# theteamatx/x-edr-trajectory-planning

Hardware: AMD Instinct MI355X
Metric: time-optimal path timings/s (7-DOF, 2000 s-samples), 1/2/4/8 MI355X + %HBM roofline (higher is better)
Workload: dtype f64

## Files before the change

### x-edr-trajectory-planning_amd/csrc/tpamd_sweep_joint.h

```cpp
#pragma once

#include <type_traits>

#include "tpamd_kernels.h"

namespace tpamd {

__device__ __forceinline__ double uniform_f64(double v) {
  const int lo = __builtin_amdgcn_readfirstlane(__double2loint(v));
  const int hi = __builtin_amdgcn_readfirstlane(__double2hiint(v));
  return __hiloint2double(hi, lo);
}
__device__ __forceinline__ double readlane_f64(double v, int lane) {
  const int lo = __builtin_amdgcn_readlane(__double2loint(v), lane);
  const int hi = __builtin_amdgcn_readlane(__double2hiint(v), lane);
  return __hiloint2double(hi, lo);
}
__device__ __forceinline__ int uniform_i32(int v) { return __builtin_amdgcn_readfirstlane(v); }
__device__ __forceinline__ int lds_word(const int *p) {
  return *(const volatile __attribute__((address_space(3))) int *)p;
}

template <int CTRL>
__device__ __forceinline__ double dpp_f64(double v) {
// ... 88 lines not shown
__device__ __forceinline__ double ordered_sum64_finite(double t, double d, const OrderedSumMasks &k) {
  double acc = t;
  const double one = 1.0;
  asm volatile("s_nop 1" ::: "memory");
  TPAMD_OSM_ROW("0x1");
  ordered_sum_carry<1>(acc);
  TPAMD_OSM_ROW("0x2");
  ordered_sum_carry<2>(acc);
  TPAMD_OSM_ROW("0x4");
  ordered_sum_carry<3>(acc);
  TPAMD_OSM_ROW("0x8");
  return acc;
}

#ifdef TPAMD_DIAG
__device__ __forceinline__ long long tpamd_stamp() {
  unsigned long long t;
  __builtin_amdgcn_sched_barrier(0);
  asm volatile("s_memtime %0\n\ts_waitcnt lgkmcnt(0)" : "=s"(t)::"memory");
  __builtin_amdgcn_sched_barrier(0);
  return (long long)t;
}
#define TPAMD_T0(var) const long long var = tpamd_stamp()
#ifdef TPAMD_DIAG_REASONS
#define TPAMD_ACC(slot, var) do { if (!((slot) == 12 || (slot) == 13 || (slot) == 17 || ((slot) >= 19 && (slot) <= 23) || (slot) == 31)) diag[slot] += tpamd_stamp() - (var); } while (0)
#else
#define TPAMD_ACC(slot, var) diag[slot] += tpamd_stamp() - (var)
#endif
#define TPAMD_CNT(slot) diag[slot] += 1
#define TPAMD_ADD(slot, v) diag[slot] += (v)
#define TPAMD_CNTX(slot) diagx[slot] += 1
#define TPAMD_T0C(var) const long long var = tpamd_stamp()
#define TPAMD_ACCC(slot, var) diag[slot] += tpamd_stamp() - (var)
#ifdef TPAMD_DIAG_LIGHT
#undef TPAMD_T0
#undef TPAMD_ACC
#define TPAMD_T0(var)
#define TPAMD_ACC(slot, var)
#endif
#else
#define TPAMD_T0(var)
#define TPAMD_ACC(slot, var)
#define TPAMD_T0C(var)
#define TPAMD_ACCC(slot, var)
#define TPAMD_CNT(slot)
#define TPAMD_ADD(slot, v)
#define TPAMD_CNTX(slot)
#endif

#ifndef TPAMD_TILE_SAMPLES
#define TPAMD_TILE_SAMPLES 32
#endif
#ifndef TPAMD_CHAIN_GUESS
#define TPAMD_CHAIN_GUESS 0
#endif
#ifndef TPAMD_CURVE_EXIT
#define TPAMD_CURVE_EXIT 1
#endif
constexpr int kTileSamples = TPAMD_TILE_SAMPLES;
template <int D>
struct TileCfg {
  static constexpr int kSamples = (D > 8 && TPAMD_TILE_SAMPLES > 16) ? 16 : TPAMD_TILE_SAMPLES;
};

typedef double f64x2 __attribute__((ext_vector_type(2)));

template <int K>
struct RegPack {
  f64x2 v;
  RegPack<K - 1> rest;
  template <int LIMIT>
  __device__ __forceinline__ void load(const f64x2 *src, int c) {
    if (c < LIMIT) v = src[c];
    rest.template load<LIMIT>(src, c + 64);
  }
  template <int LIMIT>
  __device__ __forceinline__ void store(f64x2 *dst, int c) const {
// ... 13 lines not shown
  static constexpr int RPL = (D + PARTS - 1) / PARTS;
  static constexpr int kCandLanes = 2 * D * PARTS;
  static constexpr int kRows16 = (kCandLanes + 15) / 16;
  static_assert(kCandLanes <= 64, "candidate lanes must fit one wave");
#ifndef TPAMD_CHAIN_STEPS
#define TPAMD_CHAIN_STEPS 16
#endif
  static constexpr int kChain = TPAMD_CHAIN_STEPS;
  static constexpr int GRP = 64 / kChain;
  static constexpr int CPL = (2 * D + GRP - 1) / GRP;
  static constexpr int VPL = (D + GRP - 1) / GRP;
  static constexpr unsigned long long kPart0 =
      (GRP == 4) ? 0x1111111111111111ull : ((GRP == 2) ? 0x5555555555555555ull : ~0ull);
  static_assert(GRP == 1 || GRP == 2 || GRP == 4, "chain steps must be 16, 32 or 64");
};

template <bool MAX>
__device__ __forceinline__ double ext2(double a, double b) {
  return ext2_raw<MAX>(a, b);
}

template <int D, int E = 0>
struct JointSweep {
  typedef JointLayout<D> L;
  static_assert(E == 0 || E == 2, "extra rows come as one pair");
  static constexpr int R = 2 * D + E + 2;
  static constexpr int kMt = D + E / 2;
  static constexpr int kTile = TileCfg<D>::kSamples;
  static constexpr int kChunks = kTile * R / 2;
  static constexpr int kChunksPerLane = (kChunks + 63) / 64;
#ifdef TPAMD_DIAG
  long long diag[32];
  mutable long long diagx[kDiagExt];
#endif
  int N, lane;
  double ds, two_ds;
  double *sd2;
  double *tiles;
  const uint8_t *typel;
  double *sdd_g;
  const double *m_g;
  const double *rec;
  int tag0, tag1;
  double *qd_g, *qdd_g;
  const double *aml;
  uint32_t *dirty;
  int end_idx;
  double lim;
  double chk_hi[L::RPL];
  double vel_hi;
  double vel_lo;
  int vel_mode;
  double ex_hi[E ? E : 1];
  int own_off;
  int chk_off[L::RPL];
  int vel_off;
  double row_lo, row_hi;
  double v_lim[L::CPL];
  int v_off[L::CPL];
  double vv_hi[L::VPL];
  double va_hi[L::VPL];
  int vv_off[L::VPL];

  struct Rows {
    f64x2 own;
    f64x2 chk[L::RPL];
// ... 604 lines not shown
    load_rows(idx, rows);
    if (load_cur) c.cur = uniform_f64(sd2[idx]);
    double m0, m1;
    int t0, t1;
    load_mt(idx, m0, t0);
    load_mt(idx + dir, m1, t1);
    c.m_i = uniform_f64(m0); c.m_n = uniform_f64(m1);
    c.t_i = uniform_i32(t0); c.t_n = uniform_i32(t1);
    c.nxt = uniform_f64(sd2[idx + dir]);
    c.win = -1;
    TPAMD_ACC(26, ti_);
  }

  template <bool FWD>
  __device__ __forceinline__ int add_extremal(int idx_start, Prefetch &pf, bool pair_signal = false,
                                              bool wait_pair = false) {
#define TPAMD_PAIR_SIGNAL()                                   \
  do {                                                        \
    if (pair_signal) {                                        \
      __threadfence_block();                                  \
      __syncthreads();                                        \
      pair_signal = false;                                    \
    }                                                         \
  } while (0)
    if (FWD ? !(idx_start < N - 2) : !(idx_start > 1)) {
      end_idx = idx_start;
      TPAMD_PAIR_SIGNAL();
      if (wait_pair) __syncthreads();
      return FWD ? N - 1 : 0;
    }
    Rows rows_a, rows_b;
    Carry c;
    init_carry<FWD>(idx_start, c, rows_a, pf, true);
    if (wait_pair && is_tiny(c.cur - c.m_i) && (c.t_i & kBndTrajectory) && (c.t_n & kBndTrajectory)) {
      __syncthreads();
      wait_pair = false;
    }
    bool trust = true;
    int last_win = -1;
    for (;;) {
#define TPAMD_TRY_FOLLOW()                                                                   \
  if (is_tiny(c.cur - c.m_i) && (c.t_i & kBndTrajectory) && (c.t_n & kBndTrajectory)) {      \
    TPAMD_T0(tfb_);                                                                          \
    const int run = uniform_i32(follow_boundary<FWD>(c));                                    \
    TPAMD_ACC(25, tfb_);                                                                     \
    if (run > 0) {                                                                           \
      TPAMD_CNT(8);                                                                          \
      TPAMD_PAIR_SIGNAL();                                                                   \
      if (FWD ? !(c.idx < N - 2) : !(c.idx > 1)) {                                           \
        end_idx = c.idx;                                                                     \
        return FWD ? N - 1 : 0;                                                              \
      }                                                                                      \
      init_carry<FWD>(c.idx, c, rows_a, pf, false);                                          \
      continue;                                                                              \
    }                                                                                        \
  }
#define TPAMD_TRY_CHAIN()                                                                    \
  if (c.win >= 0 && (trust || c.win == last_win)) {                                          \
    int total = 0, run, next_win;                                                            \
    bool again, curve;                                                                       \
    do {                                                                                     \
      { TPAMD_T0(tc_); run = uniform_i32(follow_chain<FWD>(c, pf, next_win, curve)); TPAMD_ACC(4, tc_); } \
      TPAMD_CNT(6);                                                                          \
      total += run;                                                                          \
      again = run == L::kChain;                                                              \
       \
// ... 66 lines not shown
    for (int top = idx_hi; top >= 1; top -= 256) {
      uint8_t ty[4];
#pragma unroll
      for (int u = 0; u < 4; u++) ty[u] = typel[max(top - 64 * u - lane, 0)];
#pragma unroll
      for (int u = 0; u < 4; u++) {
        const int idx = top - 64 * u - lane;
        const unsigned long long m = __ballot((idx >= 1) & ((ty[u] & kBndEqualsZ00) != 0));
        if (m) return top - 64 * u - (__ffsll((long long)m) - 1);
      }
    }
    return -1;
  }

#ifdef TPAMD_DIAG
  __device__ __forceinline__ int next_critical_point_literal(int idx_lo, int idx_hi) const {
    int crit = -1;
    for (int idx = idx_lo + 1; idx <= idx_hi; idx++) {
      if (crit < 0) {
        if (typel[idx] & (kBndSource | kBndTrajectory)) crit = idx;
      } else if (typel[idx] & kBndEqualsZ00) {
        crit = idx;
      }
      if (crit > 0 && !isnan(sd2[idx])) return crit;
    }
    return -1;
  }
#endif
};

constexpr int kRefitCap = 128;
constexpr int kRefitLdsBytes = kRefitCap * (4 + 8 + 8);

template <int D, int E>
struct PathBoundary {
  const JointSource &src;
  const Workspace &ws;
  int b, N, stride, lane;
  size_t pb;
  double ds, z00;
  const uint8_t *at_l;
  uint8_t *ff_l, *typel;
  bool keep;
  int *l_idx;
  double *l_val, *l_nxt;
  int count;

  __device__ __forceinline__ void append(bool need, int j, double val, double nxt) {
    const unsigned long long mask = __ballot(need);
    if (!mask) return;
    if (need) {
      const int pos = count + __popcll(mask & ((1ull << lane) - 1ull));
      l_idx[pos] = j;
      l_val[pos] = val;
      l_nxt[pos] = nxt;
    }
    count += __popcll(mask);
  }

  __device__ __forceinline__ void refit_one(int j, double sd2v, double *x, double *y) const {
    constexpr int R = 2 * D + E + 2;
    const f64x2 *rec2 = reinterpret_cast<const f64x2 *>(src.q12 + ((size_t)b * stride + j) * R);
    const double *lim_lo = src.lim + (size_t)b * 2 * (2 * D + E), *lim_hi = lim_lo + 2 * D + E;
    double a[D], bq[D];
#pragma unroll
    for (int d = 0; d < D; d++) {
      const f64x2 p = rec2[d];
      a[d] = p.x;
      bq[d] = p.y;
    }
    bool ok = true;
    if (E > 0) {
      const f64x2 ex = rec2[D];
      const double vt = ex.x * sd2v, vr = ex.y * sd2v;
      ok = !(vt + kTiny < lim_lo[2 * D] || vt - kTiny > lim_hi[2 * D]) &&
           !(vr + kTiny < lim_lo[2 * D + 1] || vr - kTiny > lim_hi[2 * D + 1]);
    }
    if (ok) find_sdd_both_joint_fixed<D>(a, bq, lim_hi, sd2v, x, y);
  }

  __device__ __forceinline__ void finalize(int j, double m, double X, double Y, double m_next) const {
    uint8_t type = kBndNone;
    if (j >= 1 && j <= N - 2) {
      const double sd2p = (m_next - m) / ds;
      const double sd2p_min = 2 * Y;
      const double sd2p_max = 2 * X;
      if (sd2p < sd2p_min) type = kBndSink;
      else if (sd2p > sd2p_max) type = kBndSource;
      if ((sd2p <= sd2p_max) && (sd2p >= sd2p_min)) type = kBndTrajectory;
    }
    if (m == z00) type |= kBndEqualsZ00;
    ws.m[pb + j] = m;
    typel[j] = type;
    if (keep) {
      ws.X[pb + j] = X;
      ws.Y[pb + j] = Y;
      ws.type[pb + j] = type;
    }
  }

  template <bool FINAL>
  __device__ __forceinline__ void flush(long long *diag) {
    TPAMD_T0(tf);
    __builtin_amdgcn_fence(__ATOMIC_ACQ_REL, "wavefront");
    __builtin_amdgcn_wave_barrier();
    const int n = count;
    for (int e = lane; e < n; e += 64) {
      const int j = l_idx[e];
      const double val = l_val[e];
      double x = 0.0, y = 0.0;
      refit_one(j, val, &x, &y);
      if (FINAL) finalize(j, val, x, y, l_nxt[e]);
      else { ws.Xz[pb + j] = x; ws.Yz[pb + j] = y; }
    }
    count = 0;
    __builtin_amdgcn_fence(__ATOMIC_ACQ_REL, "wavefront");
    __builtin_amdgcn_wave_barrier();
    if (FINAL) TPAMD_ACC(23, tf);
  }
};

template <int D, int E>
__device__ __forceinline__ void boundary_passes_for_path(const JointSource &src, const Workspace &ws, int b,
                                                         int N, int stride, int tid, uint8_t *at_l,
                                                         uint8_t *ff_l, char *scratch, uint8_t *typel,
                                                         bool keep, long long *diag) {
  TPAMD_T0C(tp0);
  const size_t pb = (size_t)b * stride;
  const int lane = tid & 63, w = tid >> 6;
  const double *m0 = ws.m0 + pb, *z0 = ws.z0 + pb, *X0 = ws.X0 + pb, *Y0 = ws.Y0 + pb;
  const double *Xz = ws.Xz + pb, *Yz = ws.Yz + pb, *fv = ws.fix_val + pb;
  PathBoundary<D, E> P{src, ws, b, N, stride, lane, pb, ws.ds[b], z0[0], at_l, ff_l, typel, keep,
                         nullptr, nullptr, nullptr, 0};
  {
    char *mine = scratch + (size_t)w * kRefitLdsBytes;
    P.l_val = reinterpret_cast<double *>(mine);
    P.l_nxt = P.l_val + kRefitCap;
    P.l_idx = reinterpret_cast<int *>(P.l_nxt + kRefitCap);
  }
  const double ds = P.ds;
  constexpr int U = 4;
  const int hi_i = N - 1;
  auto cl = [hi_i](int i) { return min(max(i, 0), hi_i); };

  for (int i = tid; i < N; i += 128) at_l[i] = ws.at0[pb + i];
  __syncthreads();
  uint8_t *iso_l = ff_l + (ff_l - at_l);
  for (int i = tid; i < N; i += 128) {
    const int a0 = at_l[cl(i - 1)], a1 = at_l[i], a2 = at_l[cl(i + 1)];
    iso_l[i] = (uint8_t)((i >= 1) & (i <= N - 2) & (a0 == 0) & (a1 != 0) & (a2 == 0));
  }
  __syncthreads();
  TPAMD_ACCC(19, tp0);

#ifndef TPAMD_BOUNDARY_FAST
#define TPAMD_BOUNDARY_FAST 1
#endif
  constexpr int UF = 17;
  const int slow_cap = ((N + 127) / 128) * 64 + 64;
  const int flag_bytes = (int)(ff_l - at_l);
  constexpr int kSegChunks = 2 * UF;
  const int nseg = (N + 62 * kSegChunks - 1) / (62 * kSegChunks);
  if (TPAMD_BOUNDARY_FAST && 3 * flag_bytes + 8 * slow_cap <= 8 * N) {
    auto fast_form = [&](auto one_segment) {
    constexpr bool kOne = decltype(one_segment)::value;
    const int nsg = kOne ? 1 : nseg;
    int *slow = reinterpret_cast<int *>(at_l + 3 * flag_bytes) + w * slow_cap;
    int nslow = 0;
    auto list_samples = [&](unsigned mask, int cb) {
#pragma unroll
      for (int u = 0; u < UF; u++) {
        const bool need = (mask >> u) & 1u;
        const unsigned long long bm = __ballot(need);
        if (bm) {
          if (need) slow[nslow + __popcll(bm & ((1ull << lane) - 1ull))] = 62 * (cb + 2 * u + w) + lane - 1;
          nslow += __popcll(bm);
        }
      }
    };
    {
      for (int seg = 0; seg < nsg; seg++) {
        const int cb = seg * kSegChunks;
        unsigned zf = 0u;
#pragma unroll
        for (int u = 0; u < UF; u++) {
          const int j = 62 * (cb + 2 * u + w) + lane - 1;
          const int jb = max(j, 1);
          zf |= (unsigned)((lane >= 1) && (lane <= 62) && (j >= 0) && (j < N) &&
                           ((iso_l[jb - 1] | iso_l[jb + 1]) != 0)) << u;
        }
        list_samples(zf, cb);
      }
      JointSweep<D, E>::wave_lds_sync();
      for (int e0 = 0; e0 < nslow; e0 += 64) {
        const bool valid = e0 + lane < nslow;
        const int j = valid ? slow[e0 + lane] : 0;
        if (P.count + 64 > kRefitCap) P.template flush<false>(diag);
        P.append(valid, j, valid ? z0[j] : 0.0, 0.0);
      }
      nslow = 0;
      P.template flush<false>(diag);
      __threadfence_block();
      __syncthreads();
      TPAMD_ACCC(20, tp0);
    }
    auto detect_one = [&](int k) {
      uint8_t flag = 0;
      if (k >= 1 && k <= N - 2) {
        const bool iso_k = iso_at(at_l, N, k), iso_km1 = iso_at(at_l, N, k - 1),
                   iso_km2 = iso_at(at_l, N, k - 2);
        const bool l_mod = iso_k || iso_km2;
        const double m_l = l_mod ? z0[k - 1] : m0[k - 1];
        const double fsmax_l = l_mod ? Xz[k - 1] : X0[k - 1];
        const double m_c = iso_km1 ? z0[k] : m0[k];
        const double X_c = iso_km1 ? Xz[k] : X0[k];
        const double Y_c = iso_km1 ? Xz[k] : Y0[k];
        const double m_r = iso_k ? z0[k + 1] : m0[k + 1];
        const double Y_r = iso_k ? Xz[k + 1] : Y0[k + 1];
        const double fsmin_r = iso_k ? Yz[k + 1] : Y0[k + 1];
        const double sd2p = (m_r - m_c) / ds;
        const double sd2p_min = 2 * Y_c;
        const double sd2p_max = 2 * X_c;
        const bool sink_or_source = (sd2p < sd2p_min) || (sd2p > sd2p_max);
        const bool skipped_sdd = (X_c > 0) && (Y_r < 0);
        const bool skipped_sd2 = (m_c > m_l - kTiny) && (m_c > m_r - kTiny);
        if ((skipped_sd2 || skipped_sdd) && sink_or_source) {
          const double fw = m_l + 2.0 * ds * fsmax_l;
          const double bw = m_r - 2.0 * ds * fsmin_r;
          double mn = z0[k];
          if (fw < mn) mn = fw;
          if (bw < mn) mn = bw;
          ws.fix_val[pb + k] = (0.0 < mn) ? mn : 0.0;
          flag = 1;
        }
      }
      ff_l[k] = flag;
    };
    auto drain_detect = [&]() {
      JointSweep<D, E>::wave_lds_sync();
      for (int e0 = 0; e0 < nslow; e0 += 64)
        if (e0 + lane < nslow) detect_one(slow[e0 + lane]);
      nslow = 0;
      JointSweep<D, E>::wave_lds_sync();
    };
    double m0c[UF], X0c[UF], Y0c[UF];
    auto load_segment = [&](int cb) {
#pragma unroll
      for (int u = 0; u < UF; u++) {
        const int c = cb + 2 * u + w;
        const int k = 62 * c + lane - 1;
        const int kc = (c >= 1 && 62 * c + 62 < N) ? k : cl(k);
        m0c[u] = m0[kc]; X0c[u] = X0[kc]; Y0c[u] = Y0[kc];
      }
    };
    const bool owner = (lane >= 1) && (lane <= 62);
    for (int seg = 0; seg < nsg; seg++) {
    const int cb = seg * kSegChunks;
    load_segment(cb);
    unsigned listed = 0u;
#pragma unroll
    for (int u = 0; u < UF; u++) {
      const int k = 62 * (cb + 2 * u + w) + lane - 1;
      const bool inside = owner && (k >= 1) && (k <= N - 2);
      const int kb = max(k, 2);
      const bool near_iso = (iso_l[kb] | iso_l[kb - 1] | iso_l[kb - 2]) != 0;
      const double m_c = m0c[u], X_c = X0c[u], Y_c = Y0c[u];
      const double m0l = dpp_f64<0x138>(m_c);
      const double m0r = dpp_f64<0x130>(m_c), Y0r = dpp_f64<0x130>(Y_c);
      const double sd2p = (m0r - m_c) / ds;
      const double sd2p_min = 2 * Y_c;
      const double sd2p_max = 2 * X_c;
      const bool sink_or_source = (sd2p < sd2p_min) || (sd2p > sd2p_max);
      const bool skipped_sdd = (X_c > 0) && (Y0r < 0);
      const bool skipped_sd2 = (m_c > m0l - kTiny) && (m_c > m0r - kTiny);
      const bool fix = (skipped_sd2 || skipped_sdd) && sink_or_source;
      const bool to_list = inside && (near_iso || fix);
      if (owner && k >= 0 && k < N && !to_list) ff_l[k] = 0;
      listed |= (unsigned)to_list << u;
    }
    list_samples(listed, cb);
    drain_detect();
    }
    __threadfence_block();
    __syncthreads();
    TPAMD_ACCC(21, tp0);

    auto final_one = [&](int j, double &m, double &X, double &Y, double &m_next) -> bool {
      bool refit = false;
      m = 0.0; X = 0.0; Y = 0.0; m_next = 0.0;
      const bool f_next = (j + 1 <= N - 2) && ff_l[j + 1];
      const bool f_self = ff_l[j];
      const bool f_prev = (j >= 1) && ff_l[j - 1];
      const bool iso_p = iso_at(at_l, N, j - 1), iso_n = iso_at(at_l, N, j + 1);
      if (f_next || (!f_self && f_prev)) {
        m = z0[j];
        if (iso_p || iso_n) { X = Xz[j]; Y = Yz[j]; }
        else refit = true;
      } else if (f_self) {
        m = fv[j];
        refit = true;
      } else if (iso_n) {
        m = z0[j]; X = Xz[j]; Y = Yz[j];
      } else if (iso_p) {
        m = z0[j]; X = Xz[j]; Y = Xz[j];
      } else {
        m = m0[j]; X = X0[j]; Y = Y0[j];
      }
      const int jn = j + 1;
      if (jn <= N - 1) {
        if (jn + 1 <= N - 2 && ff_l[jn + 1]) m_next = z0[jn];
        else if (ff_l[jn]) m_next = fv[jn];
        else if (ff_l[jn - 1]) m_next = z0[jn];
        else if (iso_at(at_l, N, jn + 1) || iso_at(at_l, N, jn - 1)) m_next = z0[jn];
        else m_next = m0[jn];
      }
      return refit;
    };
    auto drain_final = [&]() {
      JointSweep<D, E>::wave_lds_sync();
      for (int e0 = 0; e0 < nslow; e0 += 64) {
        const bool valid = e0 + lane < nslow;
        double m = 0.0, X = 0.0, Y = 0.0, m_next = 0.0;
        bool refit = false;
        int j = 0;
        if (valid) {
          j = slow[e0 + lane];
          refit = final_one(j, m, X, Y, m_next);
          if (!refit) P.finalize(j, m, X, Y, m_next);
        }
        if (P.count + 64 > kRefitCap) P.template flush<true>(diag);
        P.append(refit, j, m, m_next);
      }
      nslow = 0;
      JointSweep<D, E>::wave_lds_sync();
    };
    for (int seg = 0; seg < nsg; seg++) {
    const int cb = seg * kSegChunks;
    if (!kOne) load_segment(cb);
    unsigned listed = 0u;
#pragma unroll
    for (int u = 0; u < UF; u++) {
      const int j = 62 * (cb + 2 * u + w) + lane - 1;
      const bool mine = owner && (j >= 0) && (j < N);
      const int jb = max(j, 1);
      const bool busy = (ff_l[jb - 1] | ff_l[jb] | ff_l[jb + 1] | ff_l[jb + 2] |
                         iso_l[jb - 1] | iso_l[jb] | iso_l[jb + 1] | iso_l[jb + 2]) != 0;
      const double m0r = dpp_f64<0x130>(m0c[u]);
      if (mine && !busy) P.finalize(j, m0c[u], X0c[u], Y0c[u], (j + 1 <= N - 1) ? m0r : 0.0);
      listed |= (unsigned)(mine && busy) << u;
    }
    list_samples(listed, cb);
    drain_final();
    }
    P.template flush<true>(diag);
    __threadfence_block();
    __syncthreads();
    TPAMD_ACCC(22, tp0);
    };
    if (nseg == 1) fast_form(std::true_type{});
    else fast_form(std::false_type{});
    return;
  }

  for (int base = 64 * w; base < N; base += 128) {
    const int j = base + lane;
    const bool need = (j < N) & ((iso_l[cl(j - 1)] | iso_l[cl(j + 1)]) != 0);
    if (P.count + 64 > kRefitCap) P.template flush<false>(diag);
    P.append(need, j, need ? z0[j] : 0.0, 0.0);
  }
  P.template flush<false>(diag);
  __threadfence_block();
  __syncthreads();
  TPAMD_ACCC(20, tp0);

  for (int k0 = tid; k0 < N; k0 += 128 * U) {
    double m0l[U], m0c[U], m0r[U], z0l[U], z0c[U], z0r[U], X0l[U], X0c[U], Y0c[U], Y0r[U];
    double Xzl[U], Xzc[U], Xzr[U], Yzr[U];
#pragma unroll
    for (int u = 0; u < U; u++) {
      const int k = k0 + 128 * u;
      const int kl = cl(k - 1), kc = cl(k), kr = cl(k + 1);
      m0l[u] = m0[kl]; m0c[u] = m0[kc]; m0r[u] = m0[kr];
      X0l[u] = X0[kl]; X0c[u] = X0[kc];
      Y0c[u] = Y0[kc]; Y0r[u] = Y0[kr];
      const bool ik = iso_at(at_l, N, k), ik1 = iso_at(at_l, N, k - 1), ik2 = iso_at(at_l, N, k - 2);
      z0l[u] = (ik || ik2) ? z0[kl] : 0.0;
      z0c[u] = ik1 ? z0[kc] : 0.0;
      z0r[u] = ik ? z0[kr] : 0.0;
      Xzl[u] = (ik || ik2) ? Xz[kl] : 0.0;
      Xzc[u] = ik1 ? Xz[kc] : 0.0;
      Xzr[u] = ik ? Xz[kr] : 0.0;
      Yzr[u] = ik ? Yz[kr] : 0.0;
    }
#pragma unroll
    for (int u = 0; u < U; u++) {
      const int k = k0 + 128 * u;
      if (k >= N) continue;
      uint8_t flag = 0;
      if (k >= 1 && k <= N - 2) {
        const bool iso_k = iso_at(at_l, N, k), iso_km1 = iso_at(at_l, N, k - 1),
                   iso_km2 = iso_at(at_l, N, k - 2);
        const bool l_mod = iso_k || iso_km2;
        const double m_l = l_mod ? z0l[u] : m0l[u];
// ... 46 lines not shown
      const int j = base + 64 * u + lane;
      const bool active = j < N;
      double m = 0.0, X = 0.0, Y = 0.0, m_next = 0.0;
      bool refit = false;
      if (active) {
        const bool f_next = (j + 1 <= N - 2) && ff_l[j + 1];
        const bool f_self = ff_l[j];
        const bool f_prev = (j >= 1) && ff_l[j - 1];
        const bool iso_p = iso_at(at_l, N, j - 1), iso_n = iso_at(at_l, N, j + 1);
        if (f_next || (!f_self && f_prev)) {
          m = z0c[u];
          if (iso_p || iso_n) { X = Xzc[u]; Y = Yzc[u]; }
          else refit = true;
        } else if (f_self) {
          m = fvc[u];
          refit = true;
        } else if (iso_n) {
          m = z0c[u]; X = Xzc[u]; Y = Yzc[u];
        } else if (iso_p) {
          m = z0c[u]; X = Xzc[u]; Y = Xzc[u];
        } else {
          m = m0c[u]; X = X0c[u]; Y = Y0c[u];
        }
        const int jn = j + 1;
        if (jn <= N - 1) {
          if (jn + 1 <= N - 2 && ff_l[jn + 1]) m_next = z0n[u];
          else if (ff_l[jn]) m_next = fvn[u];
          else if (ff_l[jn - 1]) m_next = z0n[u];
          else if (iso_at(at_l, N, jn + 1) || iso_at(at_l, N, jn - 1)) m_next = z0n[u];
          else m_next = m0n[u];
        }
        if (!refit) P.finalize(j, m, X, Y, m_next);
      }
      if (P.count + 64 > kRefitCap) P.template flush<true>(diag);
      P.append(refit, j, m, m_next);
    }
  }
  P.template flush<true>(diag);
  __threadfence_block();
  __syncthreads();
  TPAMD_ACCC(22, tp0);
}

template <int D, int E = 0>
struct SweepLds {
  static constexpr int R = 2 * D + E + 2;
  static constexpr int kRingDoubles = 2 * 2 * TileCfg<D>::kSamples * R;
  __host__ __device__ static constexpr int n2(int N) { return (N + 1) & ~1; }
  __host__ __device__ static constexpr int words(int N) { return ((N + 31) / 32 + 1) & ~1; }
  __host__ __device__ static constexpr int type_bytes(int N) { return ((N + 15) / 16) * 16; }
  __host__ __device__ static constexpr size_t bytes(int N) {
    return (size_t)n2(N) * 8 + (size_t)kRingDoubles * 8 + type_bytes(N) + 64 +
           2 * (size_t)words(N) * 4 + 16 * 8 + 32;
  }
};
template <int D, int E = 0>
__host__ __device__ inline size_t sweep_joint_lds_bytes(int N) {
  return SweepLds<D, E>::bytes(N);
}

#ifndef TPAMD_SWEEP_WAVES_PER_EU
#define TPAMD_SWEEP_WAVES_PER_EU 2
#endif
#ifndef TPAMD_SWEEP_WAVES_PER_EU_WIDE
#define TPAMD_SWEEP_WAVES_PER_EU_WIDE 1
#endif
#define TPAMD_SWEEP_OCCUPANCY                                                                          \
  __attribute__((amdgpu_waves_per_eu((D > 8) ? TPAMD_SWEEP_WAVES_PER_EU_WIDE : TPAMD_SWEEP_WAVES_PER_EU, \
                                     (D > 8) ? TPAMD_SWEEP_WAVES_PER_EU_WIDE : TPAMD_SWEEP_WAVES_PER_EU)))
#ifdef TPAMD_K1_STUDY
#define TPAMD_SWEEP_STUDY_REGS __attribute__((amdgpu_num_vgpr(200)))
#else
#define TPAMD_SWEEP_STUDY_REGS
#endif
template <int D, int E = 0>
__global__ void __launch_bounds__(128) TPAMD_SWEEP_OCCUPANCY TPAMD_SWEEP_STUDY_REGS
k_sweep_joint(int stride, int max_loops, JointSource src, Workspace ws, double *t_out, double *s_out,
              double *sd_out, double *sdd_out, int32_t *lei_out, double *dtmax_out,
              int32_t *status_out, double *qd_out, double *qdd_out) {
  extern __shared__ double lds[];
  typedef JointSweep<D, E> JS;
  typedef SweepLds<D, E> LL;
  const int b = uniform_i32(path_of_block(ws, blockIdx.x));
  const int lane = threadIdx.x & 63;
  const int N = path_samples(ws, b, stride);
  const int w = uniform_i32((int)(threadIdx.x >> 6));
  const int tid = threadIdx.x;
  const size_t pb = (size_t)b * stride;
  const uint32_t bits = ws.err_bits[b];
  if (bits & kErrSkip) return;
  if (bits) {
    if (tid == 0) {
      status_out[b] = status_from_bits(bits);
      if (lei_out) lei_out[b] = 0;
      if (dtmax_out) dtmax_out[b] = -1.0;
    }
    return;
  }
#ifdef TPAMD_K1_STUDY
  unsigned long long *study = reinterpret_cast<unsigned long long *>(ws.diag) + 40960 + ((ws.keep_boundary >> 1) & 1) * 4096;
  if (tid == 0) {
    unsigned long long t;
    asm volatile("s_memrealtime %0\n\ts_waitcnt lgkmcnt(0)" : "=s"(t)::"memory");
    unsigned xcc;
    asm volatile("s_getreg_b32 %0, hwreg(HW_REG_XCC_ID)" : "=s"(xcc));
    study[2 * b] = t | ((unsigned long long)(xcc & 15u) << 60);
  }
#endif
  JS S;
  S.N = N; S.lane = lane;
  S.ds = ws.ds[b];
  S.two_ds = 2.0 * S.ds;
  S.sd2 = lds;
  double *ring = lds + LL::n2(N);
  S.tiles = ring + (size_t)w * 2 * JS::kTile * JS::R;
  uint8_t *typel = reinterpret_cast<uint8_t *>(ring + LL::kRingDoubles);
  S.typel = typel;
  int *xchg = reinterpret_cast<int *>(typel + LL::type_bytes(N));
  const int nw = LL::words(N);
  uint32_t *dirty = reinterpret_cast<uint32_t *>(xchg + 16);
  uint32_t *zero = dirty + nw;
  double *aml = reinterpret_cast<double *>(zero + nw);
  double *red = aml + 16;
  S.dirty = dirty;
  S.aml = aml;
  S.sdd_g = sdd_out + pb;
  S.m_g = ws.m + pb;
  S.rec = src.q12 + pb * JS::R;
  S.qd_g = qd_out ? qd_out + pb * D : nullptr;
  S.qdd_g = qdd_out ? qdd_out + pb * D : nullptr;
  S.end_idx = 0;
  S.tag0 = -1; S.tag1 = -1;
  double *sd2 = S.sd2;
  const double sd_start = ws.sd_start[b];
#ifdef TPAMD_DIAG
  long long(&diag)[32] = S.diag;
  long long(&diagx)[kDiagExt] = S.diagx;
  for (int k = 0; k < 32; k++) diag[k] = 0;
  for (int k = 0; k < kDiagExt; k++) diagx[k] = 0;
  volatile long long *fw_stamp = reinterpret_cast<volatile long long *>(red + 2);
#define TPAMD_DIAG_PTR S.diag
#else
#define TPAMD_DIAG_PTR nullptr
#endif
  boundary_passes_for_path<D, E>(src, ws, b, N, stride, tid, reinterpret_cast<uint8_t *>(sd2),
                           reinterpret_cast<uint8_t *>(sd2) + LL::type_bytes(N),
                           reinterpret_cast<char *>(ring), typel, (ws.keep_boundary & 1) != 0,
                           TPAMD_DIAG_PTR);
  constexpr int C = 2 * D + E;
  const double *lim_lo = src.lim + (size_t)b * 2 * C, *lim_hi = lim_lo + C;
  {
    typedef JointLayout<D> L;
    const double kInf = __longlong_as_double(0x7ff0000000000000LL);
    const bool is_cand = lane < L::kCandLanes;
    const int c = is_cand ? lane / L::PARTS : 0;
    const int p = lane % L::PARTS;
    const int r = c >> 1;
    S.own_off = r;
    S.lim = is_cand ? ((c & 1) ? lim_hi[r] : lim_lo[r]) : qnan();
#pragma unroll
    for (int k = 0; k < L::RPL; k++) {
      int j = p + k * L::PARTS;
      if (j >= D) j = (p < D) ? p : 0;
      S.chk_off[k] = j;
      S.chk_hi[k] = lim_hi[j];
    }
    const bool is_vel = lane < D;
    S.vel_off = is_vel ? lane : 0;
    S.vel_hi = is_vel ? lim_hi[D + lane] : kInf;
    S.vel_lo = is_vel ? 0.0 : -kInf;
    S.vel_mode = 0;
    if (E > 0) {
      if (lane >= D && lane < D + E) {
        S.vel_off = D;
        S.vel_mode = 1 + (lane - D);
        S.vel_hi = lim_hi[2 * D + (lane - D)];
        S.vel_lo = lim_lo[2 * D + (lane - D)];
      }
#pragma unroll
      for (int k = 0; k < (E ? E : 1); k++) S.ex_hi[k] = lim_hi[2 * D + k];
    }
  }
  S.row_lo = (lane < C) ? lim_lo[lane] : 0.0;
  S.row_hi = (lane < C) ? lim_hi[lane] : 0.0;
  {
    typedef JointLayout<D> L;
    const double kInf = __longlong_as_double(0x7ff0000000000000LL);
    const int p = lane & (L::GRP - 1);
#pragma unroll
    for (int i = 0; i < L::CPL; i++) {
      const int cand = p + L::GRP * i;
      const bool has = cand < 2 * D;
      const int row = has ? (cand >> 1) : 0;
      S.v_off[i] = row;
      S.v_lim[i] = has ? ((cand & 1) ? lim_hi[row] : lim_lo[row]) : qnan();
    }
#pragma unroll
    for (int i = 0; i < L::VPL; i++) {
      const int row = p + L::GRP * i;
      const bool has = row < D;
      S.vv_off[i] = has ? row : 0;
      S.vv_hi[i] = has ? lim_hi[D + row] : kInf;
      S.va_hi[i] = has ? lim_hi[row] : kInf;
    }
  }

  for (int i = tid; i < N; i += 128) {
    sd2[i] = qnan();
    S.sdd_g[i] = qnan();
  }
  for (int i = tid; i < 2 * nw; i += 128) dirty[i] = 0u;
  if (tid < D) aml[tid] = ws.amax ? ws.amax[(size_t)b * D + tid] : 0.0;
  __syncthreads();
  if (tid == 0) {
    xchg[2] = 0;
    xchg[6] = 0;
    sd2[0] = sd_start * sd_start;
    sd2[N - 1] = 0;
  }
  __syncthreads();

  int status = 0;
  int iforw_lo = 0, iback_hi = N - 1, iback_lo, iforw_hi, icrit, icrit_lo, icrit_hi;
  typename JS::Prefetch pf;
  pf.tag = -1;
  TPAMD_T0C(t_all);
  int emitted_hi = 0, upper_lo = N;
#ifndef TPAMD_FIRST_PAIR_CONCURRENT
#define TPAMD_FIRST_PAIR_CONCURRENT 1
#endif
#ifndef TPAMD_EMIT_IN_LOOP
#define TPAMD_EMIT_IN_LOOP 1
#endif
  bool first_pair_in_order = !TPAMD_FIRST_PAIR_CONCURRENT;
  if (TPAMD_FIRST_PAIR_CONCURRENT) {
    if (w == 0) {
      const int r = S.template add_extremal<false>(iback_hi, pf);
      if (lane == 0) { xchg[0] = r; xchg[7] = S.end_idx; }
    } else {
      const int r = S.template add_extremal<true>(iforw_lo, pf);
      if (lane == 0) { xchg[1] = r; xchg[8] = S.end_idx; }
    }
    __threadfence_block();
    __syncthreads();
    const int end_b = uniform_i32(xchg[7]), end_f = uniform_i32(xchg[8]);
    if (!(end_f + 70 < end_b)) {
      first_pair_in_order = true;
      for (int i = tid; i < N; i += 128) {
        sd2[i] = qnan();
        S.sdd_g[i] = qnan();
      }
      __syncthreads();
      if (tid == 0) {
        sd2[0] = sd_start * sd_start;
        sd2[N - 1] = 0;
      }
      __threadfence_block();
      __syncthreads();
// ... 431 lines not shown
```

Before: 2.129 million.

## Overlap boundary-pass loads with prologue and reuse classification verdicts

For the 7-DOF single-segment case, the boundary pass now issues its m/X/Y chunk loads before the at0 copy and streams later chunks in a sliding window. It computes the sink/source/trajectory verdict once in the detect loop and reuses it at finalize time, and moves the zero-fit stage after detection. Kernel prologue work is hoisted into callbacks so it overlaps the boundary-pass latency: lane-constant limit loads, the first tile prefetch and the early LDS/global initialisation stores. A VGPR ceiling is also set for the flagship instance. In exchange the code is more complex, register pressure rises from the held verdict and chunk arrays, and a reordered zfit stage is a correctness risk.

Result: no change. 2.109 million (-1.0%).

```diff
diff --git a/x-edr-trajectory-planning_amd/csrc/tpamd_sweep_joint.h b/x-edr-trajectory-planning_amd/csrc/tpamd_sweep_joint.h
--- a/x-edr-trajectory-planning_amd/csrc/tpamd_sweep_joint.h
+++ b/x-edr-trajectory-planning_amd/csrc/tpamd_sweep_joint.h
@@ -144,6 +144,7 @@
 #define TPAMD_CNTX(slot) diagx[slot] += 1
 #define TPAMD_T0C(var) const long long var = tpamd_stamp()
 #define TPAMD_ACCC(slot, var) diag[slot] += tpamd_stamp() - (var)
+#define TPAMD_ACCX(slot, var) diagx[slot] += tpamd_stamp() - (var)
 #ifdef TPAMD_DIAG_LIGHT
 #undef TPAMD_T0
 #undef TPAMD_ACC
@@ -155,6 +156,7 @@
 #define TPAMD_ACC(slot, var)
 #define TPAMD_T0C(var)
 #define TPAMD_ACCC(slot, var)
+#define TPAMD_ACCX(slot, var)
 #define TPAMD_CNT(slot)
 #define TPAMD_ADD(slot, v)
 #define TPAMD_CNTX(slot)
@@ -234,6 +236,7 @@
 #ifdef TPAMD_DIAG
   long long diag[32];
   mutable long long diagx[kDiagExt];
+  long long t_first;
 #endif
   int N, lane;
   double ds, two_ds;
@@ -904,6 +907,9 @@
     Rows rows_a, rows_b;
     Carry c;
     init_carry<FWD>(idx_start, c, rows_a, pf, true);
+#ifdef TPAMD_DIAG
+    if (diagx[14] == 0) diagx[14] = tpamd_stamp() - t_first;
+#endif
     if (wait_pair && is_tiny(c.cur - c.m_i) && (c.t_i & kBndTrajectory) && (c.t_n & kBndTrajectory)) {
       __syncthreads();
       wait_pair = false;
@@ -1036,6 +1042,9 @@
 constexpr int kRefitCap = 128;
 constexpr int kRefitLdsBytes = kRefitCap * (4 + 8 + 8);
 
+#ifndef TPAMD_BOUNDARY_FAST
+#define TPAMD_BOUNDARY_FAST 1
+#endif
 template <int D, int E>
 struct PathBoundary {
   const JointSource &src;
@@ -1083,16 +1092,25 @@
     if (ok) find_sdd_both_joint_fixed<D>(a, bq, lim_hi, sd2v, x, y);
   }
 
+  static __device__ __forceinline__ uint8_t classify(bool below, bool above, bool within) {
+    uint8_t type = kBndNone;
+    if (below) type = kBndSink;
+    else if (above) type = kBndSource;
+    if (within) type = kBndTrajectory;
+    return type;
+  }
   __device__ __forceinline__ void finalize(int j, double m, double X, double Y, double m_next) const {
     uint8_t type = kBndNone;
     if (j >= 1 && j <= N - 2) {
       const double sd2p = (m_next - m) / ds;
       const double sd2p_min = 2 * Y;
       const double sd2p_max = 2 * X;
-      if (sd2p < sd2p_min) type = kBndSink;
-      else if (sd2p > sd2p_max) type = kBndSource;
-      if ((sd2p <= sd2p_max) && (sd2p >= sd2p_min)) type = kBndTrajectory;
-    }
+      type = classify(sd2p < sd2p_min, sd2p > sd2p_max, (sd2p <= sd2p_max) && (sd2p >= sd2p_min));
+    }
+    store_final(j, m, X, Y, type);
+  }
+  __device__ __forceinline__ void store_final(int j, double m, double X, double Y, uint8_t inner) const {
+    uint8_t type = (j >= 1 && j <= N - 2) ? inner : (uint8_t)kBndNone;
     if (m == z00) type |= kBndEqualsZ00;
     ws.m[pb + j] = m;
     typel[j] = type;
@@ -1104,8 +1122,8 @@
   }
 
   template <bool FINAL>
-  __device__ __forceinline__ void flush(long long *diag) {
-    TPAMD_T0(tf);
+  __device__ __forceinline__ void flush(long long *diag, long long *diagx) {
+    TPAMD_T0C(tf);
     __builtin_amdgcn_fence(__ATOMIC_ACQ_REL, "wavefront");
     __builtin_amdgcn_wave_barrier();
     const int n = count;
@@ -1120,15 +1138,31 @@
     count = 0;
     __builtin_amdgcn_fence(__ATOMIC_ACQ_REL, "wavefront");
     __builtin_amdgcn_wave_barrier();
-    if (FINAL) TPAMD_ACC(23, tf);
+    if (FINAL) TPAMD_ACCC(23, tf);
+    else TPAMD_ACCX(12, tf);
   }
 };
 
-template <int D, int E>
+#if defined(TPAMD_INST_D) && defined(TPAMD_INST_E)
+#if TPAMD_INST_D == 7 && TPAMD_INST_E == 0
+#define TPAMD_BP_FLAGSHIP_INSTANCE 1
+#endif
+#endif
+#ifndef TPAMD_BP_FLAGSHIP_INSTANCE
+#define TPAMD_BP_FLAGSHIP_INSTANCE 0
+#endif
+#ifndef TPAMD_BP_SEGMENT_FIRST
+#define TPAMD_BP_SEGMENT_FIRST TPAMD_BP_FLAGSHIP_INSTANCE
+#endif
+#ifndef TPAMD_BP_REUSE_VERDICT
+#define TPAMD_BP_REUSE_VERDICT TPAMD_BP_FLAGSHIP_INSTANCE
+#endif
+template <int D, int E, class AfterLoads, class BeforeClose>
 __device__ __forceinline__ void boundary_passes_for_path(const JointSource &src, const Workspace &ws, int b,
                                                          int N, int stride, int tid, uint8_t *at_l,
                                                          uint8_t *ff_l, char *scratch, uint8_t *typel,
-                                                         bool keep, long long *diag) {
+                                                         bool keep, long long *diag, long long *diagx,
+                                                         AfterLoads &&after_loads, BeforeClose &&before_close) {
   TPAMD_T0C(tp0);
   const size_t pb = (size_t)b * stride;
   const int lane = tid & 63, w = tid >> 6;
@@ -1147,7 +1181,45 @@
   const int hi_i = N - 1;
   auto cl = [hi_i](int i) { return min(max(i, 0), hi_i); };
 
-  for (int i = tid; i < N; i += 128) at_l[i] = ws.at0[pb + i];
+  constexpr int UF = 17;
+  constexpr int kSegChunks = 2 * UF;
+  const int slow_cap = ((N + 127) / 128) * 64 + 64;
+  const int flag_bytes = (int)(ff_l - at_l);
+  const int nseg = (N + 62 * kSegChunks - 1) / (62 * kSegChunks);
+  const bool fast = TPAMD_BOUNDARY_FAST && 3 * flag_bytes + 8 * slow_cap <= 8 * N;
+  double m0c[UF], X0c[UF], Y0c[UF];
+#ifndef TPAMD_BP_WINDOW
+#define TPAMD_BP_WINDOW 7
+#endif
+  constexpr int kWindow = TPAMD_BP_WINDOW;
+  auto load_chunks = [&](int cb, int u0, int u1) {
+#pragma unroll
+    for (int u = 0; u < UF; u++) {
+      if (u < u0 || u >= u1) continue;
+      const int c = cb + 2 * u + w;
+      const int k = 62 * c + lane - 1;
+      const int kc = (c >= 1 && 62 * c + 62 < N) ? k : cl(k);
+      m0c[u] = m0[kc]; X0c[u] = X0[kc]; Y0c[u] = Y0[kc];
+    }
+  };
+  auto load_segment = [&](int cb) { load_chunks(cb, 0, UF); };
+  const bool early = TPAMD_BP_SEGMENT_FIRST && fast && nseg == 1;
+  if (early) {
+    uint8_t a0[UF];
+#pragma unroll
+    for (int u = 0; u < UF; u++) a0[u] = ws.at0[pb + min(tid + 128 * u, hi_i)];
+    __builtin_amdgcn_sched_barrier(0);
+    load_chunks(0, 0, kWindow);
+    __builtin_amdgcn_sched_barrier(0);
+    after_loads();
+    __builtin_amdgcn_sched_barrier(0);
+#pragma unroll
+    for (int u = 0; u < UF; u++)
+      if (tid + 128 * u < N) at_l[tid + 128 * u] = a0[u];
+  } else {
+    for (int i = tid; i < N; i += 128) at_l[i] = ws.at0[pb + i];
+    after_loads();
+  }
   __syncthreads();
   uint8_t *iso_l = ff_l + (ff_l - at_l);
   for (int i = tid; i < N; i += 128) {
@@ -1157,17 +1229,10 @@
   __syncthreads();
   TPAMD_ACCC(19, tp0);
 
-#ifndef TPAMD_BOUNDARY_FAST
-#define TPAMD_BOUNDARY_FAST 1
-#endif
-  constexpr int UF = 17;
-  const int slow_cap = ((N + 127) / 128) * 64 + 64;
-  const int flag_bytes = (int)(ff_l - at_l);
-  constexpr int kSegChunks = 2 * UF;
-  const int nseg = (N + 62 * kSegChunks - 1) / (62 * kSegChunks);
-  if (TPAMD_BOUNDARY_FAST && 3 * flag_bytes + 8 * slow_cap <= 8 * N) {
+  if (fast) {
     auto fast_form = [&](auto one_segment) {
     constexpr bool kOne = decltype(one_segment)::value;
+    constexpr bool kEarly = kOne && TPAMD_BP_SEGMENT_FIRST;
     const int nsg = kOne ? 1 : nseg;
     int *slow = reinterpret_cast<int *>(at_l + 3 * flag_bytes) + w * slow_cap;
     int nslow = 0;
@@ -1182,7 +1247,7 @@
         }
       }
     };
-    {
+    auto zfit_stage = [&]() {
       for (int seg = 0; seg < nsg; seg++) {
         const int cb = seg * kSegChunks;
         unsigned zf = 0u;
@@ -1199,15 +1264,16 @@
       for (int e0 = 0; e0 < nslow; e0 += 64) {
         const bool valid = e0 + lane < nslow;
         const int j = valid ? slow[e0 + lane] : 0;
-        if (P.count + 64 > kRefitCap) P.template flush<false>(diag);
+        if (P.count + 64 > kRefitCap) P.template flush<false>(diag, diagx);
         P.append(valid, j, valid ? z0[j] : 0.0, 0.0);
       }
       nslow = 0;
-      P.template flush<false>(diag);
+      P.template flush<false>(diag, diagx);
       __threadfence_block();
       __syncthreads();
       TPAMD_ACCC(20, tp0);
-    }
+    };
+    if (!kEarly) zfit_stage();
     auto detect_one = [&](int k) {
       uint8_t flag = 0;
       if (k >= 1 && k <= N - 2) {
@@ -1241,30 +1307,33 @@
       ff_l[k] = flag;
     };
     auto drain_detect = [&]() {
+      TPAMD_T0C(td);
       JointSweep<D, E>::wave_lds_sync();
       for (int e0 = 0; e0 < nslow; e0 += 64)
         if (e0 + lane < nslow) detect_one(slow[e0 + lane]);
       nslow = 0;
       JointSweep<D, E>::wave_lds_sync();
-    };
-    double m0c[UF], X0c[UF], Y0c[UF];
-    auto load_segment = [&](int cb) {
-#pragma unroll
-      for (int u = 0; u < UF; u++) {
-        const int c = cb + 2 * u + w;
-        const int k = 62 * c + lane - 1;
-        const int kc = (c >= 1 && 62 * c + 62 < N) ? k : cl(k);
-        m0c[u] = m0[kc]; X0c[u] = X0[kc]; Y0c[u] = Y0[kc];
-      }
+      TPAMD_ACCX(10, td);
     };
     const bool owner = (lane >= 1) && (lane <= 62);
+    unsigned long long verdict = 0ull;
+    unsigned eqz = 0u, listed_early = 0u;
     for (int seg = 0; seg < nsg; seg++) {
     const int cb = seg * kSegChunks;
-    load_segment(cb);
+    if (!kEarly) load_segment(cb);
+#ifdef TPAMD_DIAG
+    {
+      TPAMD_T0C(tw);
+      asm volatile("s_waitcnt vmcnt(0)" ::: "memory");
+      TPAMD_ACCX(9, tw);
+    }
+#endif
     unsigned listed = 0u;
+    int ln = lane;
+    if (kEarly) asm volatile("" : "+v"(ln));
 #pragma unroll
     for (int u = 0; u < UF; u++) {
-      const int k = 62 * (cb + 2 * u + w) + lane - 1;
+      const int k = 62 * (cb + 2 * u + w) + ln - 1;
       const bool inside = owner && (k >= 1) && (k <= N - 2);
       const int kb = max(k, 2);
       const bool near_iso = (iso_l[kb] | iso_l[kb - 1] | iso_l[kb - 2]) != 0;
@@ -1274,16 +1343,43 @@
       const double sd2p = (m0r - m_c) / ds;
       const double sd2p_min = 2 * Y_c;
       const double sd2p_max = 2 * X_c;
-      const bool sink_or_source = (sd2p < sd2p_min) || (sd2p > sd2p_max);
+      const bool below = sd2p < sd2p_min, above = sd2p > sd2p_max;
+      const bool sink_or_source = below || above;
+      if (kEarly || (kOne && TPAMD_BP_REUSE_VERDICT)) {
+        const uint8_t t = PathBoundary<D, E>::classify(below, above, (sd2p <= sd2p_max) && (sd2p >= sd2p_min));
+        verdict |= (unsigned long long)((t & kBndTrajectory) ? 3 : t) << (2 * u);
+        asm volatile("" : "+v"(verdict));
+      }
+      if (kEarly) {
+        eqz |= (unsigned)(m_c == P.z00) << u;
+        asm volatile("" : "+v"(eqz));
+        if (owner && k >= 0 && k < N) ws.m[pb + k] = m_c;
+      }
       const bool skipped_sdd = (X_c > 0) && (Y0r < 0);
       const bool skipped_sd2 = (m_c > m0l - kTiny) && (m_c > m0r - kTiny);
       const bool fix = (skipped_sd2 || skipped_sdd) && sink_or_source;
       const bool to_list = inside && (near_iso || fix);
       if (owner && k >= 0 && k < N && !to_list) ff_l[k] = 0;
       listed |= (unsigned)to_list << u;
-    }
-    list_samples(listed, cb);
-    drain_detect();
+      if (kEarly) asm volatile("" : "+v"(listed));
+      if (kEarly && (u & 1)) __builtin_amdgcn_sched_barrier(0);
+      if (kEarly && u + kWindow < UF) {
+        __builtin_amdgcn_sched_barrier(0);
+        load_chunks(0, u + kWindow, u + kWindow + 1);
+        __builtin_amdgcn_sched_barrier(0);
+      }
+    }
+    if (kEarly) {
+      listed_early = listed;
+    } else {
+      list_samples(listed, cb);
+      drain_detect();
+    }
+    }
+    if (kEarly) {
+      zfit_stage();
+      list_samples(listed_early, 0);
+      drain_detect();
     }
     __threadfence_block();
     __syncthreads();
@@ -1321,6 +1417,7 @@
       return refit;
     };
     auto drain_final = [&]() {
+      TPAMD_T0C(td);
       JointSweep<D, E>::wave_lds_sync();
       for (int e0 = 0; e0 < nslow; e0 += 64) {
         const bool valid = e0 + lane < nslow;
@@ -1332,11 +1429,12 @@
           refit = final_one(j, m, X, Y, m_next);
           if (!refit) P.finalize(j, m, X, Y, m_next);
         }
-        if (P.count + 64 > kRefitCap) P.template flush<true>(diag);
+        if (P.count + 64 > kRefitCap) P.template flush<true>(diag, diagx);
         P.append(refit, j, m, m_next);
       }
       nslow = 0;
       JointSweep<D, E>::wave_lds_sync();
+      TPAMD_ACCX(11, td);
     };
     for (int seg = 0; seg < nsg; seg++) {
     const int cb = seg * kSegChunks;
@@ -1350,13 +1448,31 @@
       const bool busy = (ff_l[jb - 1] | ff_l[jb] | ff_l[jb + 1] | ff_l[jb + 2] |
                          iso_l[jb - 1] | iso_l[jb] | iso_l[jb + 1] | iso_l[jb + 2]) != 0;
       const double m0r = dpp_f64<0x130>(m0c[u]);
-      if (mine && !busy) P.finalize(j, m0c[u], X0c[u], Y0c[u], (j + 1 <= N - 1) ? m0r : 0.0);
+      if (kEarly) {
+        const unsigned v = (unsigned)(verdict >> (2 * u)) & 3u;
+        if (mine && !busy) {
+          uint8_t type = (j >= 1 && j <= N - 2) ? (uint8_t)(v == 3u ? kBndTrajectory : v) : (uint8_t)kBndNone;
+          if ((eqz >> u) & 1u) type |= kBndEqualsZ00;
+          typel[j] = type;
+          if (keep) {
+            ws.X[pb + j] = X0[j];
+            ws.Y[pb + j] = Y0[j];
+            ws.type[pb + j] = type;
+          }
+        }
+      } else if (kOne && TPAMD_BP_REUSE_VERDICT) {
+        const unsigned v = (unsigned)(verdict >> (2 * u)) & 3u;
+        if (mine && !busy) P.store_final(j, m0c[u], X0c[u], Y0c[u], (uint8_t)(v == 3u ? kBndTrajectory : v));
+      } else {
+        if (mine && !busy) P.finalize(j, m0c[u], X0c[u], Y0c[u], (j + 1 <= N - 1) ? m0r : 0.0);
+      }
       listed |= (unsigned)(mine && busy) << u;
     }
     list_samples(listed, cb);
     drain_final();
     }
-    P.template flush<true>(diag);
+    P.template flush<true>(diag, diagx);
+    before_close();
     __threadfence_block();
     __syncthreads();
     TPAMD_ACCC(22, tp0);
@@ -1369,10 +1485,10 @@
   for (int base = 64 * w; base < N; base += 128) {
     const int j = base + lane;
     const bool need = (j < N) & ((iso_l[cl(j - 1)] | iso_l[cl(j + 1)]) != 0);
-    if (P.count + 64 > kRefitCap) P.template flush<false>(diag);
+    if (P.count + 64 > kRefitCap) P.template flush<false>(diag, diagx);
     P.append(need, j, need ? z0[j] : 0.0, 0.0);
   }
-  P.template flush<false>(diag);
+  P.template flush<false>(diag, diagx);
   __threadfence_block();
   __syncthreads();
   TPAMD_ACCC(20, tp0);
@@ -1485,11 +1601,12 @@
         }
         if (!refit) P.finalize(j, m, X, Y, m_next);
       }
-      if (P.count + 64 > kRefitCap) P.template flush<true>(diag);
+      if (P.count + 64 > kRefitCap) P.template flush<true>(diag, diagx);
       P.append(refit, j, m, m_next);
     }
   }
-  P.template flush<true>(diag);
+  P.template flush<true>(diag, diagx);
+  before_close();
   __threadfence_block();
   __syncthreads();
   TPAMD_ACCC(22, tp0);
@@ -1526,8 +1643,18 @@
 #else
 #define TPAMD_SWEEP_STUDY_REGS
 #endif
+#if !defined(TPAMD_SWEEP_MAX_VGPRS) && defined(TPAMD_INST_D) && defined(TPAMD_INST_E)
+#if TPAMD_INST_D == 7 && TPAMD_INST_E == 0
+#define TPAMD_SWEEP_MAX_VGPRS 208
+#endif
+#endif
+#ifdef TPAMD_SWEEP_MAX_VGPRS
+#define TPAMD_SWEEP_REG_CEILING __attribute__((amdgpu_num_vgpr((TPAMD_SWEEP_MAX_VGPRS) / 2)))
+#else
+#define TPAMD_SWEEP_REG_CEILING
+#endif
 template <int D, int E = 0>
-__global__ void __launch_bounds__(128) TPAMD_SWEEP_OCCUPANCY TPAMD_SWEEP_STUDY_REGS
+__global__ void __launch_bounds__(128) TPAMD_SWEEP_OCCUPANCY TPAMD_SWEEP_STUDY_REGS TPAMD_SWEEP_REG_CEILING
 k_sweep_joint(int stride, int max_loops, JointSource src, Workspace ws, double *t_out, double *s_out,
               double *sd_out, double *sdd_out, int32_t *lei_out, double *dtmax_out,
               int32_t *status_out, double *qd_out, double *qdd_out) {
@@ -1593,77 +1720,109 @@
   for (int k = 0; k < kDiagExt; k++) diagx[k] = 0;
   volatile long long *fw_stamp = reinterpret_cast<volatile long long *>(red + 2);
 #define TPAMD_DIAG_PTR S.diag
+#define TPAMD_DIAGX_PTR S.diagx
 #else
 #define TPAMD_DIAG_PTR nullptr
-#endif
-  boundary_passes_for_path<D, E>(src, ws, b, N, stride, tid, reinterpret_cast<uint8_t *>(sd2),
-                           reinterpret_cast<uint8_t *>(sd2) + LL::type_bytes(N),
-                           reinterpret_cast<char *>(ring), typel, (ws.keep_boundary & 1) != 0,
-                           TPAMD_DIAG_PTR);
+#define TPAMD_DIAGX_PTR nullptr
+#endif
+#ifndef TPAMD_PROLOGUE_OVERLAP
+#define TPAMD_PROLOGUE_OVERLAP (TPAMD_BP_FLAGSHIP_INSTANCE ? 7 : 0)
+#endif
   constexpr int C = 2 * D + E;
   const double *lim_lo = src.lim + (size_t)b * 2 * C, *lim_hi = lim_lo + C;
-  {
-    typedef JointLayout<D> L;
-    const double kInf = __longlong_as_double(0x7ff0000000000000LL);
-    const bool is_cand = lane < L::kCandLanes;
-    const int c = is_cand ? lane / L::PARTS : 0;
-    const int p = lane % L::PARTS;
-    const int r = c >> 1;
-    S.own_off = r;
-    S.lim = is_cand ? ((c & 1) ? lim_hi[r] : lim_lo[r]) : qnan();
-#pragma unroll
-    for (int k = 0; k < L::RPL; k++) {
-      int j = p + k * L::PARTS;
-      if (j >= D) j = (p < D) ? p : 0;
-      S.chk_off[k] = j;
-      S.chk_hi[k] = lim_hi[j];
-    }
-    const bool is_vel = lane < D;
-    S.vel_off = is_vel ? lane : 0;
-    S.vel_hi = is_vel ? lim_hi[D + lane] : kInf;
-    S.vel_lo = is_vel ? 0.0 : -kInf;
-    S.vel_mode = 0;
-    if (E > 0) {
-      if (lane >= D && lane < D + E) {
-        S.vel_off = D;
-        S.vel_mode = 1 + (lane - D);
-        S.vel_hi = lim_hi[2 * D + (lane - D)];
-        S.vel_lo = lim_lo[2 * D + (lane - D)];
-      }
-#pragma unroll
-      for (int k = 0; k < (E ? E : 1); k++) S.ex_hi[k] = lim_hi[2 * D + k];
-    }
-  }
-  S.row_lo = (lane < C) ? lim_lo[lane] : 0.0;
-  S.row_hi = (lane < C) ? lim_hi[lane] : 0.0;
-  {
-    typedef JointLayout<D> L;
-    const double kInf = __longlong_as_double(0x7ff0000000000000LL);
-    const int p = lane & (L::GRP - 1);
-#pragma unroll
-    for (int i = 0; i < L::CPL; i++) {
-      const int cand = p + L::GRP * i;
-      const bool has = cand < 2 * D;
-      const int row = has ? (cand >> 1) : 0;
-      S.v_off[i] = row;
-      S.v_lim[i] = has ? ((cand & 1) ? lim_hi[row] : lim_lo[row]) : qnan();
-    }
-#pragma unroll
-    for (int i = 0; i < L::VPL; i++) {
-      const int row = p + L::GRP * i;
-      const bool has = row < D;
-      S.vv_off[i] = has ? row : 0;
-      S.vv_hi[i] = has ? lim_hi[D + row] : kInf;
-      S.va_hi[i] = has ? lim_hi[row] : kInf;
-    }
-  }
-
-  for (int i = tid; i < N; i += 128) {
-    sd2[i] = qnan();
-    S.sdd_g[i] = qnan();
-  }
-  for (int i = tid; i < 2 * nw; i += 128) dirty[i] = 0u;
-  if (tid < D) aml[tid] = ws.amax ? ws.amax[(size_t)b * D + tid] : 0.0;
+  auto load_lane_constants = [&]() {
+    {
+      typedef JointLayout<D> L;
+      const double kInf = __longlong_as_double(0x7ff0000000000000LL);
+      const bool is_cand = lane < L::kCandLanes;
+      const int c = is_cand ? lane / L::PARTS : 0;
+      const int p = lane % L::PARTS;
+      const int r = c >> 1;
+      S.own_off = r;
+      S.lim = is_cand ? ((c & 1) ? lim_hi[r] : lim_lo[r]) : qnan();
+#pragma unroll
+      for (int k = 0; k < L::RPL; k++) {
+        int j = p + k * L::PARTS;
+        if (j >= D) j = (p < D) ? p : 0;
+        S.chk_off[k] = j;
+        S.chk_hi[k] = lim_hi[j];
+      }
+      const bool is_vel = lane < D;
+      S.vel_off = is_vel ? lane : 0;
+      S.vel_hi = is_vel ? lim_hi[D + lane] : kInf;
+      S.vel_lo = is_vel ? 0.0 : -kInf;
+      S.vel_mode = 0;
+      if (E > 0) {
+        if (lane >= D && lane < D + E) {
+          S.vel_off = D;
+          S.vel_mode = 1 + (lane - D);
+          S.vel_hi = lim_hi[2 * D + (lane - D)];
+          S.vel_lo = lim_lo[2 * D + (lane - D)];
+        }
+#pragma unroll
+        for (int k = 0; k < (E ? E : 1); k++) S.ex_hi[k] = lim_hi[2 * D + k];
+      }
+    }
+    S.row_lo = (lane < C) ? lim_lo[lane] : 0.0;
+    S.row_hi = (lane < C) ? lim_hi[lane] : 0.0;
+    {
+      typedef JointLayout<D> L;
+      const double kInf = __longlong_as_double(0x7ff0000000000000LL);
+      const int p = lane & (L::GRP - 1);
+#pragma unroll
+      for (int i = 0; i < L::CPL; i++) {
+        const int cand = p + L::GRP * i;
+        const bool has = cand < 2 * D;
+        const int row = has ? (cand >> 1) : 0;
+        S.v_off[i] = row;
+        S.v_lim[i] = has ? ((cand & 1) ? lim_hi[row] : lim_lo[row]) : qnan();
+      }
+#pragma unroll
+      for (int i = 0; i < L::VPL; i++) {
+        const int row = p + L::GRP * i;
+        const bool has = row < D;
+        S.vv_off[i] = has ? row : 0;
+        S.vv_hi[i] = has ? lim_hi[D + row] : kInf;
+        S.va_hi[i] = has ? lim_hi[row] : kInf;
+      }
+    }
+  };
+  auto early_stores = [&](bool with_sd2) {
+    for (int i = tid; i < N; i += 128) {
+      if (with_sd2) sd2[i] = qnan();
+      S.sdd_g[i] = qnan();
+    }
+    for (int i = tid; i < 2 * nw; i += 128) dirty[i] = 0u;
+    if (tid < D) aml[tid] = ws.amax ? ws.amax[(size_t)b * D + tid] : 0.0;
+  };
+  typename JS::Prefetch pf;
+  pf.tag = -1;
+  const int first_tile = (w == 0) ? (N - 1) / JS::kTile : 0;
+  boundary_passes_for_path<D, E>(
+      src, ws, b, N, stride, tid, reinterpret_cast<uint8_t *>(sd2),
+      reinterpret_cast<uint8_t *>(sd2) + LL::type_bytes(N), reinterpret_cast<char *>(ring), typel,
+      (ws.keep_boundary & 1) != 0, TPAMD_DIAG_PTR, TPAMD_DIAGX_PTR,
+      [&]() {
+        if (TPAMD_PROLOGUE_OVERLAP & 2) early_stores(false);
+      },
+      [&]() {
+        if (TPAMD_PROLOGUE_OVERLAP & 4)
+          pf.r.template load<JS::kChunks>(
+              reinterpret_cast<const f64x2 *>(S.rec + (size_t)first_tile * JS::kTile * JS::R), lane);
+        if (TPAMD_PROLOGUE_OVERLAP & 1) load_lane_constants();
+      });
+  TPAMD_T0C(t_pro);
+  if (!(TPAMD_PROLOGUE_OVERLAP & 1)) load_lane_constants();
+  if (TPAMD_PROLOGUE_OVERLAP & 4) {
+    pf.m = S.m_g[min(first_tile * JS::kTile + (lane & (JS::kTile - 1)), N - 1)];
+    pf.tag = first_tile;
+  }
+
+  if (TPAMD_PROLOGUE_OVERLAP & 2) {
+    for (int i = tid; i < N; i += 128) sd2[i] = qnan();
+  } else {
+    early_stores(true);
+  }
   __syncthreads();
   if (tid == 0) {
     xchg[2] = 0;
@@ -1672,11 +1831,13 @@
     sd2[N - 1] = 0;
   }
   __syncthreads();
+  TPAMD_ACCX(13, t_pro);
+#ifdef TPAMD_DIAG
+  S.t_first = tpamd_stamp();
+#endif
 
   int status = 0;
   int iforw_lo = 0, iback_hi = N - 1, iback_lo, iforw_hi, icrit, icrit_lo, icrit_hi;
-  typename JS::Prefetch pf;
-  pf.tag = -1;
   TPAMD_T0C(t_all);
   int emitted_hi = 0, upper_lo = N;
 #ifndef TPAMD_FIRST_PAIR_CONCURRENT
```
